# johannah/drqv2

Hardware: AMD Instinct MI355X
Metric: agent updates/sec (batch=256, 9x84x84 obs) (higher is better)
Workload: dtype f32; 1 GPU; cheetah_run batch_size=256/GPU (256 global) 9x84x84 u8 obs, A=6, feature_dim=50, hidden_dim=1024, fp32, use_tb=True; parallelism=dp1, global_batch=256

## Files before the change

drqv2_amd/csrc/conv1aug.hip:

```cpp
#include "common.h"
#include "internal.h"
#include "replay_device.h"
#include "wino_u.h"

namespace {

constexpr int H = 84, C = 9, PAD = 4, S = 92, HW = H * H;
constexpr int HO = 41, PO = HO * HO;
constexpr int NBAND = 5;
constexpr int MAXR = 9;
constexpr int NROWS = 2 * MAXR + 1;
constexpr int SROWS = NROWS + 2;
constexpr int XPL = 42;
constexpr int XPITCH = 2 * XPL;
constexpr int HQ = H / 4;
constexpr int CP = 5, NS = CP * 9;
constexpr int XS_FLOATS = C * NROWS * XPITCH;
constexpr int U8_DWORDS = C * SROWS * HQ;
constexpr int NDMA = (U8_DWORDS + 63) / 64;
constexpr int U8_ALLOC = NDMA * 64;
constexpr int NTHR = 256;
constexpr int NWAVE = NTHR / 64;
constexpr int MAXU = 64;
constexpr int FG = 3, GC = C / FG;
constexpr int LDS_BYTES = (XS_FLOATS + U8_ALLOC + H + (2 + FG) * MAXU) * 4;
static_assert(2 * LDS_BYTES <= 160 * 1024, "two workgroups share a CU's LDS");

struct Conv1AugArgs {
  const uint8_t* obs[2];
  const long* fidx[2];
  const uint8_t* ring_first;
  long ring_R, ring_N;
  const float* shift[2];
  const float* base;
  const float* w;
  const float* bias;
  float* xaug;
  float* y;
  int n, n_store;
  unsigned y_bytes;
  int stagger;
  const float* wino_w[3];
  float* wino_u;
  int n_rider;
};

typedef float f32x2 __attribute__((ext_vector_type(2)));
typedef __bf16 bf16x8_c1 __attribute__((ext_vector_type(8)));
typedef unsigned u32x4_c1 __attribute__((ext_vector_type(4)));
typedef unsigned u32x2_c1 __attribute__((ext_vector_type(2)));

__device__ __forceinline__ unsigned pack_bf16_c1(float lo, float hi) {
  typedef __bf16 bf16x2_c1 __attribute__((ext_vector_type(2)));
  const bf16x2_c1 v = {(__bf16)lo, (__bf16)hi};
  return __builtin_bit_cast(unsigned, v);
}

__device__ __forceinline__ float div255(float v) {
  const float r = 1.0f / 255.0f;
  const float q = __fmul_rn(v, r);
  const float e = __fmaf_rn(-q, 255.0f, v);
  return __fmaf_rn(e, r, q);
}

template <bool BF = false, bool YN = false>
__global__ __launch_bounds__(NTHR, 2 * NTHR / 256) void conv1_aug_kernel(Conv1AugArgs a) {
#pragma clang fp contract(off)
  extern __shared__ __attribute__((aligned(16))) float smem[];
  typedef __attribute__((address_space(3))) void* lds_ptr_t;
  typedef const __attribute__((address_space(1))) void* glb_ptr_t;
  float* xs = smem;
  unsigned* u8w = reinterpret_cast<unsigned*>(smem + XS_FLOATS);
  const uint8_t* u8b = reinterpret_cast<const uint8_t*>(u8w);
  float* bg = smem + XS_FLOATS + U8_ALLOC;
  float* shs = bg + H;
  int* fof = reinterpret_cast<int*>(shs + 2 * MAXU);
  const int tid = threadIdx.x;
  const int lane = tid & 63, wid = __builtin_amdgcn_readfirstlane(tid >> 6);
  const int col = lane & 31, half = lane >> 5;
  if ((int)blockIdx.x < a.n_rider) {
    const int job = blockIdx.x;
    wino_u_image<false>(a.wino_w[job >> 1], job & 1, smem, a.wino_u + (size_t)job * 16384, tid);
    return;
  }
  const int bid = (int)blockIdx.x - a.n_rider;
  const int units = 2 * a.n * NBAND;
  const int G = (int)gridDim.x - a.n_rider;

  if (tid < H) bg[tid] = a.base[tid];
  if (tid >= 128 && tid < 128 + MAXU) {
    const int k = tid - 128, uu = bid + k * G;
    if (uu < units) {
      const int f = uu / NBAND;
      const int view = f >= a.n ? 1 : 0, fb = f - view * a.n;
      shs[2 * k + 0] = a.shift[view][2 * fb + 0];
      shs[2 * k + 1] = a.shift[view][2 * fb + 1];
      const long f0 = a.fidx[view] ? a.fidx[view][fb] : fb;
      if (a.ring_first) {
        const long S = a.ring_R * a.ring_N;
        long sl[FG];
        ring_stack_slots(a.ring_first, a.ring_R, a.ring_N, f0 < 0 ? 0 : (f0 < S ? f0 : S - 1), sl);
#pragma unroll
        for (int g = 0; g < FG; ++g) fof[FG * k + g] = (int)sl[g];
      } else {
#pragma unroll
        for (int g = 0; g < FG; ++g) fof[FG * k + g] = (int)(FG * f0 + g);
      }
    }
  }
  float wreg[NS];
#pragma unroll
  for (int c = 0; c < CP; ++c)
#pragma unroll
    for (int t = 0; t < 9; ++t) {
      const int cin = 2 * c + half;
      wreg[c * 9 + t] = cin < C ? a.w[(col * C + cin) * 9 + t] : 0.f;
    }
  bf16x8_c1 wfb[9];
  if constexpr (BF) {
#pragma unroll
    for (int t = 0; t < 9; ++t) {
      float wv[8];
#pragma unroll
      for (int j = 0; j < 8; ++j) {
        const int cin = 8 * half + j;
        wv[j] = cin < C ? a.w[(col * C + (cin < C ? cin : 0)) * 9 + t] : 0.f;
      }
      const u32x4_c1 pk = {pack_bf16_c1(wv[0], wv[1]), pack_bf16_c1(wv[2], wv[3]), pack_bf16_c1(wv[4], wv[5]),
                           pack_bf16_c1(wv[6], wv[7])};
      wfb[t] = __builtin_bit_cast(bf16x8_c1, pk);
    }
  }
  float breg[16];
#pragma unroll
  for (int r = 0; r < 16; ++r) breg[r] = a.bias[(r & 3) + 8 * (r >> 2) + 4 * half];
  const __amdgpu_buffer_rsrc_t yrsrc = __builtin_amdgcn_make_buffer_rsrc((void*)a.y, 0, a.y_bytes, 0x00020000);
  __syncthreads();

  const float sc = (float)(2.0 / (double)S);
  auto cl = [&](int v) { v -= PAD; return v < 0 ? 0 : (v > H - 1 ? H - 1 : v); };
  auto coordv = [&](int k, float sh, float& fl) {
    const float g = bg[k] + sh;
    const float v = ((g + 1.f) * (float)S - 1.f) / 2.f;
    fl = floorf(v);
    return v;
  };

  struct Unit {
    int f, r0, R, i0, nr, sy_lo, nsrc, fo[FG];
    float shx, shy;
  };
  auto make_unit = [&](int k) {
    const int u = bid + k * G;
    Unit q;
    q.f = u / NBAND;
    const int band = u - q.f * NBAND;
    q.r0 = band == 0 ? 0 : 9 + 8 * (band - 1);
    q.R = band == 0 ? 9 : 8;
    q.i0 = 2 * q.r0;
    q.nr = 2 * q.R + 1 + (band == NBAND - 1 ? 1 : 0);
    q.shx = shs[2 * k + 0] * sc;
    q.shy = shs[2 * k + 1] * sc;
#pragma unroll
    for (int g = 0; g < FG; ++g) q.fo[g] = fof[FG * k + g];
    float fa, fbb;
    coordv(q.i0, q.shy, fa);
    coordv(q.i0 + q.nr - 1, q.shy, fbb);
    q.sy_lo = cl((int)fa);
    q.nsrc = cl((int)fbb + 1) - q.sy_lo + 1;
    return q;
  };
  auto dma_src = [&](const Unit& q) {
    const int view = q.f >= a.n ? 1 : 0;
    const uint8_t* src3[FG];
#pragma unroll
    for (int g = 0; g < FG; ++g) src3[g] = a.obs[view] + (long)q.fo[g] * GC * HW;
    for (int k = wid; k < NDMA; k += NWAVE) {
      int e = k * 64 + lane;
      e = e < U8_DWORDS ? e : U8_DWORDS - 1;
      const int rowid = e / HQ, qd = e - rowid * HQ;
      const int ch = rowid / SROWS, r = rowid - ch * SROWS;
      const int rr = r < q.nsrc ? r : q.nsrc - 1;
      const int grp = ch / GC;
      const uint8_t* src = grp == 0 ? src3[0] : (grp == 1 ? src3[1] : src3[2]);
      const unsigned* g = reinterpret_cast<const unsigned*>(src + (ch - grp * GC) * HW + (q.sy_lo + rr) * H) + qd;
      __builtin_amdgcn_global_load_lds((glb_ptr_t)g, (lds_ptr_t)(u8w + k * 64), 4, 0, 0);
    }
  };

  const int nmine = bid < units ? (units - 1 - bid) / G + 1 : 0;
  Unit cur{};
  if (nmine > 0) {
    cur = make_unit(0);
    dma_src(cur);
  }
  if (a.stagger) {
    const unsigned hwid = __builtin_amdgcn_s_getreg((4 << 0) | (0 << 6) | (31 << 11));
    if (hwid & 1u) {
      for (int q = 0; q < a.stagger; ++q) __builtin_amdgcn_s_sleep(127);
    }
  }
  for (int k = 0; k < nmine; ++k) {
    asm volatile("s_waitcnt vmcnt(0)" ::: "memory");
    __syncthreads();

    {
      const bool store = cur.f < a.n_store;
      const __amdgpu_buffer_rsrc_t xrs = __builtin_amdgcn_make_buffer_rsrc(
          (void*)(a.xaug + (long)cur.f * C * HW), 0, store ? (unsigned)(C * HW * 4) : 0u, 0x00020000);
      constexpr int RPP = NTHR / H;
      const int j = tid % H, r3 = tid / H;
      if (r3 < RPP) {
        float fx;
        const float ix = coordv(j, cur.shx, fx);
        const int x0 = (int)fx;
        const float wx1 = ix - fx, wx0 = (fx + 1.f) - ix;
        const bool okx0 = x0 >= 0 && x0 < S, okx1 = x0 + 1 >= 0 && x0 + 1 < S;
        const int sx0 = cl(x0), sx1 = cl(x0 + 1);
        const int xcol = (j & 1) * XPL + (j >> 1);
        for (int il = r3; il < cur.nr; il += RPP) {
          const int i = cur.i0 + il;
          float fy;
          const float iy = coordv(i, cur.shy, fy);
          const int y0 = (int)fy;
          const float wy1 = iy - fy, wy0 = (fy + 1.f) - iy;
          const bool oky0 = y0 >= 0 && y0 < S, oky1 = y0 + 1 >= 0 && y0 + 1 < S;
          const int sy0 = cl(y0), sy1 = cl(y0 + 1);
          const float w00 = okx0 && oky0 ? wx0 * wy0 : 0.f, w01 = okx1 && oky0 ? wx1 * wy0 : 0.f;
          const float w10 = okx0 && oky1 ? wx0 * wy1 : 0.f, w11 = okx1 && oky1 ? wx1 * wy1 : 0.f;
          const int o00 = (sy0 - cur.sy_lo) * H + sx0, o01 = (sy0 - cur.sy_lo) * H + sx1;
          const int o10 = (sy1 - cur.sy_lo) * H + sx0, o11 = (sy1 - cur.sy_lo) * H + sx1;
          const int xo = il * XPITCH + xcol;
          const int go = (i * H + j) * 4;
          uint8_t tap[C][4];
#pragma unroll
          for (int ch = 0; ch < C; ++ch) {
            const uint8_t* s8 = u8b + ch * SROWS * H;
            tap[ch][0] = s8[o00]; tap[ch][1] = s8[o01]; tap[ch][2] = s8[o10]; tap[ch][3] = s8[o11];
          }
          const f32x2 W00 = {w00, w00}, W01 = {w01, w01}, W10 = {w10, w10}, W11 = {w11, w11};
          const f32x2 R255 = {1.0f / 255.0f, 1.0f / 255.0f}, N255 = {-255.0f, -255.0f}, MH = {-0.5f, -0.5f};
#pragma unroll
          for (int cp = 0; cp < C / 2; ++cp) {
            const int c0 = 2 * cp, c1 = 2 * cp + 1;
            f32x2 p0 = (f32x2){(float)tap[c0][0], (float)tap[c1][0]} * W00;
            f32x2 p1 = (f32x2){(float)tap[c0][1], (float)tap[c1][1]} * W01;
            f32x2 p2 = (f32x2){(float)tap[c0][2], (float)tap[c1][2]} * W10;
            f32x2 p3 = (f32x2){(float)tap[c0][3], (float)tap[c1][3]} * W11;
            asm volatile("" : "+v"(p0), "+v"(p1), "+v"(p2), "+v"(p3));
            f32x2 v = p0 + p1;
            asm volatile("" : "+v"(v));
            v = v + p2;
            asm volatile("" : "+v"(v));
            v = v + p3;
            asm volatile("" : "+v"(v));
            f32x2 q = v * R255;
            asm volatile("" : "+v"(q));
            const f32x2 e = __builtin_elementwise_fma(q, N255, v);
            q = __builtin_elementwise_fma(e, R255, q);
            asm volatile("" : "+v"(q));
            q = q + MH;
            xs[c0 * NROWS * XPITCH + xo] = q[0];
            xs[c1 * NROWS * XPITCH + xo] = q[1];
            __builtin_amdgcn_raw_buffer_store_b32(__float_as_uint(q[0]), xrs, go, c0 * HW * 4, 0);
            __builtin_amdgcn_raw_buffer_store_b32(__float_as_uint(q[1]), xrs, go, c1 * HW * 4, 0);
          }
          {
            constexpr int ch = C - 1;
            float p0 = (float)tap[ch][0] * w00, p1 = (float)tap[ch][1] * w01, p2 = (float)tap[ch][2] * w10,
                  p3 = (float)tap[ch][3] * w11;
            asm volatile("" : "+v"(p0), "+v"(p1), "+v"(p2), "+v"(p3));
            float v = p0 + p1;
            v = v + p2;
            v = v + p3;
            v = __fsub_rn(div255(v), 0.5f);
            xs[ch * NROWS * XPITCH + xo] = v;
            __builtin_amdgcn_raw_buffer_store_b32(__float_as_uint(v), xrs, go, ch * HW * 4, 0);
          }
        }
      }
    }
    __syncthreads();

    const Unit done = cur;
    if (k + 1 < nmine) {
      cur = make_unit(k + 1);
      dma_src(cur);
    }

    const int npix = done.R * HO;
    const int ntiles = (npix + 31) >> 5;
    auto load_group = [&](float (&dst)[9], const float* xb, int c) {
      const int ch = (c == CP - 1) ? (C - 1) : 2 * c + half;
      const float* xc = xb + ch * (NROWS * XPITCH);
#pragma unroll
      for (int ky = 0; ky < 3; ++ky) {
        dst[ky * 3 + 0] = xc[ky * XPITCH];
        dst[ky * 3 + 1] = xc[ky * XPITCH + XPL];
        dst[ky * 3 + 2] = xc[ky * XPITCH + 1];
      }
    };
    for (int tile = wid; tile < (wid >= 4 ? 0 : ntiles); tile += 4) {
      const int p0 = tile * 32 + col;
      const int p = p0 < npix ? p0 : npix - 1;
      const int oyl = p / HO, ox = p - oyl * HO;
      const float* xb = xs + (2 * oyl) * XPITCH + ox;
      f32x16 acc;
#pragma unroll
      for (int r = 0; r < 16; ++r) acc[r] = breg[r];
      if constexpr (BF) {
        const float* xj[8];
#pragma unroll
        for (int j = 0; j < 8; ++j) xj[j] = xb + (half ? C - 1 : j) * (NROWS * XPITCH);
#pragma unroll
        for (int t = 0; t < 9; ++t) {
          const int ky = t / 3, kx = t - 3 * ky;
          const int off = ky * XPITCH + (kx == 1 ? XPL : 0) + (kx == 2 ? 1 : 0);
          float v[8];
#pragma unroll
          for (int j = 0; j < 8; ++j) v[j] = xj[j][off];
          const u32x4_c1 pk = {pack_bf16_c1(v[0], v[1]), pack_bf16_c1(v[2], v[3]), pack_bf16_c1(v[4], v[5]),
                               pack_bf16_c1(v[6], v[7])};
          acc = __builtin_amdgcn_mfma_f32_32x32x16_bf16(wfb[t], __builtin_bit_cast(bf16x8_c1, pk), acc, 0, 0, 0);
        }
      } else {
      float X[2][9];
      load_group(X[0], xb, 0);
#pragma unroll
      for (int c = 0; c < CP; ++c) {
        acc = __builtin_amdgcn_mfma_f32_32x32x2f32(wreg[c * 9], X[c & 1][0], acc, 0, 0, 0);
        __builtin_amdgcn_sched_barrier(0);
        if (c + 1 < CP) load_group(X[(c + 1) & 1], xb, c + 1);
        __builtin_amdgcn_sched_barrier(0);
#pragma unroll
        for (int t = 1; t < 9; ++t)
          acc = __builtin_amdgcn_mfma_f32_32x32x2f32(wreg[c * 9 + t], X[c & 1][t], acc, 0, 0, 0);
        __builtin_amdgcn_sched_barrier(0);
      }
      }
      const int oy = done.r0 + oyl;
      if constexpr (YN) {
        const int yo = p0 < npix ? (((done.f * HO + oy) * HO + ox) * 16 + half * 2) * 4 : (int)0x80000000u;
#pragma unroll
        for (int g4 = 0; g4 < 4; ++g4) {
          float v[4];
#pragma unroll
          for (int e = 0; e < 4; ++e) v[e] = acc[4 * g4 + e] > 0.f ? acc[4 * g4 + e] : 0.f;
          const u32x2_c1 o = {pack_bf16_c1(v[0], v[1]), pack_bf16_c1(v[2], v[3])};
          __builtin_amdgcn_raw_buffer_store_b64(o, yrsrc, yo, g4 * 16, 0);
        }
        continue;
      }
      const int yoff = p0 < npix ? (((done.f * 32 + 4 * half) * HO + oy) * HO + ox) * 4 : (int)0x80000000u;
#pragma unroll
      for (int r = 0; r < 16; ++r) {
        const float v = acc[r] > 0.f ? acc[r] : 0.f;
        __builtin_amdgcn_raw_buffer_store_b32(__float_as_uint(v), yrsrc, yoff, ((r & 3) + 8 * (r >> 2)) * PO * 4, 0);
      }
    }
  }
}

}

int drq_conv1_aug_fwd_any(int bf_mma, const uint8_t* obs, const float* shift, const uint8_t* obs1, const float* shift1,
                          const float* base_grid, const float* w, const float* bias, float* xaug, float* y, int n,
                          int n_store, hipStream_t st, const float* const* wino_w, float* wino_u, const long* fidx0,
                          const long* fidx1, const uint8_t* ring_first, long ring_R, long ring_N) {
  if (!obs || !shift || !obs1 || !shift1 || !base_grid || !w || !bias || !y || n <= 0 || n_store < 0 || n_store > 2 * n)
    return DRQ_EARG;
  if (n_store > 0 && !xaug) return DRQ_EARG;
  if (((uintptr_t)obs & 3) || ((uintptr_t)obs1 & 3)) return DRQ_EARG;
  if (ring_first && (!fidx0 || !fidx1 || obs != obs1 || ring_R <= 0 || ring_N <= 0 || ring_R > INT32_MAX / ring_N))
    return DRQ_EARG;
  const size_t yb = (size_t)2 * n * 32 * PO * (bf_mma == 2 ? 2 : 4);
  if (yb >= (1ull << 31) || (bf_mma == 2 && ((uintptr_t)y & 15))) return DRQ_EARG;
  Conv1AugArgs a{};
  a.obs[0] = obs; a.obs[1] = obs1;
  a.fidx[0] = fidx0; a.fidx[1] = fidx1;
  a.ring_first = ring_first; a.ring_R = ring_R; a.ring_N = ring_N;
  a.shift[0] = shift; a.shift[1] = shift1;
  a.base = base_grid; a.w = w; a.bias = bias; a.xaug = xaug; a.y = y;
  a.n = n; a.n_store = n_store; a.y_bytes = (unsigned)yb; a.stagger = 1;
  if (wino_w && wino_u) {
    for (int l = 0; l < 3; ++l) a.wino_w[l] = wino_w[l];
    a.wino_u = wino_u;
    a.n_rider = 6;
  }
  static bool attr_set_dev[kMaxDevices] = {};
  bool& attr_set = attr_set_dev[drq_device()];
  if (!attr_set) {
    hipError_t e = hipFuncSetAttribute((const void*)conv1_aug_kernel<false>, hipFuncAttributeMaxDynamicSharedMemorySize,
                                       LDS_BYTES);
    if (e == hipSuccess)
      e = hipFuncSetAttribute((const void*)conv1_aug_kernel<true>, hipFuncAttributeMaxDynamicSharedMemorySize, LDS_BYTES);
    if (e == hipSuccess)
      e = hipFuncSetAttribute((const void*)conv1_aug_kernel<true, true>, hipFuncAttributeMaxDynamicSharedMemorySize,
                              LDS_BYTES);
    if (e != hipSuccess) return (int)e;
    attr_set = true;
  }
  const long units = (long)2 * n * NBAND;
  long blocks = units;
  const long cap = 2L * drq_num_cus();
  if (blocks > cap) blocks = cap;
  if (blocks * MAXU < units) blocks = (units + MAXU - 1) / MAXU;
  blocks += a.n_rider;
  if (bf_mma == 2) hipLaunchKernelGGL((conv1_aug_kernel<true, true>), dim3((unsigned)blocks), dim3(NTHR), LDS_BYTES, st, a);
  else if (bf_mma) hipLaunchKernelGGL((conv1_aug_kernel<true>), dim3((unsigned)blocks), dim3(NTHR), LDS_BYTES, st, a);
  else hipLaunchKernelGGL((conv1_aug_kernel<false>), dim3((unsigned)blocks), dim3(NTHR), LDS_BYTES, st, a);
  DRQ_LAUNCH_CHECK();
  return DRQ_OK;
}

DRQ_API int drq_conv1_aug_fwd(const uint8_t* obs, const float* shift, const uint8_t* obs1, const float* shift1,
                              const float* base_grid, const float* w, const float* bias, float* xaug, float* y, int n,
                              int n_store, hipStream_t st) {
  return drq_conv1_aug_fwd_any(0, obs, shift, obs1, shift1, base_grid, w, bias, xaug, y, n, n_store, st, nullptr, nullptr,
                               nullptr, nullptr, nullptr, 0, 0);
}

DRQ_API int drq_conv1_aug_fwd_indexed(const uint8_t* frames, const long* idx, const float* shift, const uint8_t* frames1,
                                      const long* idx1, const float* shift1, const float* base_grid, const float* w,
                                      const float* bias, float* xaug, float* y, int n, int n_store, hipStream_t st) {
  if (!idx || !idx1) return DRQ_EARG;
  return drq_conv1_aug_fwd_any(0, frames, shift, frames1, shift1, base_grid, w, bias, xaug, y, n, n_store, st, nullptr,
                               nullptr, idx, idx1, nullptr, 0, 0);
}

DRQ_API int drq_conv1_aug_fwd_frames(const uint8_t* frames, const uint8_t* first, long R, long N, const long* idx,
                                     const float* shift, const long* idx1, const float* shift1, const float* base_grid,
                                     const float* w, const float* bias, float* xaug, float* y, int n, int n_store,
                                     hipStream_t st) {
  if (!first || !idx || !idx1) return DRQ_EARG;
  return drq_conv1_aug_fwd_any(0, frames, shift, frames, shift1, base_grid, w, bias, xaug, y, n, n_store, st, nullptr,
                               nullptr, idx, idx1, first, R, N);
}

DRQ_API int drq_conv1_aug_fwd_frames_bf16(const uint8_t* frames, const uint8_t* first, long R, long N, const long* idx,
                                          const float* shift, const long* idx1, const float* shift1,
                                          const float* base_grid, const float* w, const float* bias, float* xaug,
                                          float* y, int n, int n_store, hipStream_t st) {
  if (!first || !idx || !idx1) return DRQ_EARG;
  return drq_conv1_aug_fwd_any(1, frames, shift, frames, shift1, base_grid, w, bias, xaug, y, n, n_store, st, nullptr,
                               nullptr, idx, idx1, first, R, N);
}

DRQ_API int drq_conv1_aug_fwd_bf16(const uint8_t* obs, const float* shift, const uint8_t* obs1, const float* shift1,
                                   const float* base_grid, const float* w, const float* bias, float* xaug, float* y,
                                   int n, int n_store, hipStream_t st) {
  return drq_conv1_aug_fwd_any(1, obs, shift, obs1, shift1, base_grid, w, bias, xaug, y, n, n_store, st, nullptr, nullptr,
                               nullptr, nullptr, nullptr, 0, 0);
}

DRQ_API int drq_conv1_aug_fwd_bf16_nhwc(const uint8_t* obs, const float* shift, const uint8_t* obs1, const float* shift1,
                                        const float* base_grid, const float* w, const float* bias, float* xaug,
                                        void* y_nhwc, int n, int n_store, hipStream_t st) {
  return drq_conv1_aug_fwd_any(2, obs, shift, obs1, shift1, base_grid, w, bias, xaug, (float*)y_nhwc, n, n_store, st,
                               nullptr, nullptr, nullptr, nullptr, nullptr, 0, 0);
}
```

drqv2_amd/replay.py:

```python
import collections
import datetime
import pathlib

import numpy as np
import torch

from . import _lib
from . import episodes as _episodes
from ._lib import launch, ptr
from .checkpoint import check_state, host

ExportReport = collections.namedtuple("ExportReport", "files episodes transitions next_row zero_length headless open short")
ExportReport.__doc__ = """What export_episodes() did: files (the paths written, in order), episodes and transitions (how many
of each they hold), next_row (pass it as start_row next time), and how many runs were left out as zero_length, headless,
open and short (drqv2_amd.episodes.plan_export says what each means)."""
FillReport = collections.namedtuple("FillReport", "episodes transitions rows pad_rows")
FillReport.__doc__ = """What add_episodes() did: episodes and transitions placed, rows added to the ring (T grew by that), and
pad_rows, the reset rows that fill the shorter lanes (counted over all environments)."""


class IndexedBatch(tuple):

    def __new__(cls, frames, obs_idx, action, reward, discount, next_idx):
        self = super().__new__(cls, (obs_idx, action, reward, discount, next_idx))
# ... 98 lines not shown
    if isinstance(priority_alpha, bool) or not (0.0 < a <= 1.0):
        raise ValueError(f"priority_alpha {priority_alpha!r}: None or a float in (0, 1]")
    if not (store.priority_beta >= 0.0) or not (0.0 < store.priority_eps < float("inf")):
        raise ValueError("priority_beta must be >= 0 and priority_eps > 0")
    return a


def _priority_tree(store, slots, alpha):
    _on_gpu(store, "prioritized replay keeps its sum tree")
    store.priority_alpha = alpha
    store.tree_leaves = 1 << max(0, slots - 1).bit_length()
    store.tree = torch.zeros(2 * store.tree_leaves, dtype=torch.float64, device=store.device)
    store.tree[0] = 1.0
    store._pbufs = {}


class BatchIterator:

    def __init__(self, draw, store=None):
        self._draw = draw
        self._store = store
        self._ahead = None
        self._drawn = None

    def __iter__(self):
        return self

    def __next__(self):
        b, self._ahead = self._ahead, None
        return b if b is not None else self._draw()

    def prefetch(self):
        if self._ahead is None:
            self._ahead = self._draw()
            if self._store is not None:
                self._drawn = (self._store.last_index, self._store.last_steps)

    def peek(self):
        self.prefetch()
        return self._ahead

    def state_dict(self):
        store = self._store
        if store is None:
            raise _lib.DrqError("BatchIterator.state_dict(): this iterator was built without a store: only the iterators "
                                "of VecDeviceReplay / VecFrameReplay can be saved")
        sd = {"format": 1, "kind": "BatchIterator", "pending": self._ahead is not None}
        if self._ahead is None:
            return sd
        if not store.indexed:
            raise _lib.DrqError("BatchIterator.state_dict(): a pending materialised batch (indexed=False) cannot be saved")
        if store.device.type == "cuda":
            torch.cuda.synchronize(store.device)
        b = self._ahead
        sd.update(index=host(self._drawn[0]), steps=host(self._drawn[1]), action=host(b[1]), reward=host(b[2]),
                  discount=host(b[3]), prioritized=isinstance(b, PrioritizedBatch))
        if sd["prioritized"]:
            sd.update(weights=host(b.weights), stamp=int(b._stamp))
        return sd

    def load_state_dict(self, sd):
        store = self._store
        if store is None:
            raise _lib.DrqError("BatchIterator.load_state_dict(): this iterator was built without a store")
        check_state(self, sd, kind="BatchIterator")
        if not sd.get("pending"):
            self._ahead = self._drawn = None
            return
        index = sd.get("index")
        if not torch.is_tensor(index) or index.dim() != 2 or index.shape[0] != 3:
            raise ValueError("BatchIterator.load_state_dict(): a pending batch needs its index tensor [3, B]")
        B, per = int(index.shape[1]), bool(sd.get("prioritized"))
        want = {"index": ((3, B), torch.int64), "steps": ((B,), torch.int32), "action": ((B, store.A), torch.float32),
                "reward": ((B, 1), torch.float32), "discount": ((B, 1), torch.float32)}
        if per:
            want["weights"] = ((B,), torch.float32)
        check_state(self, sd, tensors=want, kind="BatchIterator")
        if per != (store.tree is not None) or not store.indexed:
            raise ValueError("BatchIterator.load_state_dict(): the saved batch is "
                             f"{'prioritized' if per else 'uniform'} and indexed, the store is not")
        if B and not (0 <= int(index.min()) and int(index.max()) < store.R * store.N):
            raise ValueError(f"BatchIterator.load_state_dict(): slots outside the ring of {store.R * store.N}")
        dev = store.device
        idx, steps, act, rew, disc = (sd[k].to(dev) for k in ("index", "steps", "action", "reward", "discount"))
        batch = store._batch(per, idx, act, rew, disc)
        if per:
            batch._per(store, idx[2], sd["weights"].to(dev))
            batch._stamp = int(sd["stamp"])
        self._ahead, self._drawn = batch, (idx, steps)
        store.last_index, store.last_steps = idx, steps


class DeviceReplay:
    def __init__(self, capacity_steps, obs_shape, action_dim, nstep, discount, device, seed=None, indexed=False,
                 priority_alpha=None, priority_beta=0.4, priority_eps=1e-6, single_frames=False, check_stacks=True):
        self.device = torch.device(device)
        self.obs_shape = tuple(int(s) for s in obs_shape)
        self.single_frames, self.check_stacks = bool(single_frames), bool(check_stacks)
        if self.single_frames and self.obs_shape != (9, 84, 84):
            raise ValueError(f"obs_shape {self.obs_shape}: a single-frame store stacks three (3, 84, 84) frames")
        self.stack_bytes = int(np.prod(self.obs_shape))
        self.frame_bytes = self.stack_bytes // 3 if self.single_frames else self.stack_bytes
        if self.frame_bytes % 16:
            raise ValueError("frame size must be a multiple of 16 bytes")
        self.A = int(action_dim)
        self.nstep = int(nstep)
        self.gamma = float(discount)
        self.capacity = int(capacity_steps)
        dev = self.device
        self.frames = torch.empty((self.capacity, self.frame_bytes), dtype=torch.uint8, device=dev)
        self.action = torch.zeros((self.capacity, self.A), dtype=torch.float32, device=dev)
        self.reward = torch.zeros((self.capacity,), dtype=torch.float32, device=dev)
        self.discount = torch.ones((self.capacity,), dtype=torch.float32, device=dev)
        self.first = torch.zeros((self.capacity,), dtype=torch.uint8, device=dev) if self.single_frames else None
        self.episodes = []
        self._head = 0
        self.rng = np.random.RandomState(seed)
        self._out = {}
        self.indexed = bool(indexed)
        self._ibufs = {}
        self._placements = 0
        self.n_valid = 0
        alpha = _priority_args(self, priority_alpha, priority_beta, priority_eps)
        if alpha is not None:
            _priority_tree(self, self.capacity, alpha)

    def __len__(self):
        return sum(n - 1 for _, n in self.episodes)

    def _place(self, n):
        if n > self.capacity:
            raise ValueError(f"episode of {n} steps exceeds the store ({self.capacity})")
        start = self._head if self._head + n <= self.capacity else 0
        end = start + n
        clear = lambda e: e[0] + e[1] <= start or e[0] >= end
        evicted = [e for e in self.episodes if not clear(e)]
        self.episodes = [e for e in self.episodes if clear(e)]
        self._head = end
        return start, evicted

    def _fill(self, lo, hi, mode):
        launch("drq_per_fill", ptr(self.tree), self.tree_leaves, lo, hi, mode, device=self.device)

    def _place_priorities(self, start, n, evicted):
        for s, m in evicted:
            self._fill(s, s + m, 0)
        self._fill(start, start + n, 0)
        if n - 1 >= self.nstep:
            self._fill(start + 1, start + n - self.nstep + 1, 1)
        self.n_valid = sum(m - self.nstep for _, m in self.episodes if m - 1 >= self.nstep)

    def add_episode(self, episode):
        if self.single_frames:
            obs = newest_frames(episode["observation"], self.check_stacks)
        else:
            obs = np.ascontiguousarray(episode["observation"])
            if obs.dtype != np.uint8 or int(np.prod(obs.shape[1:])) != self.frame_bytes:
                raise ValueError("observation must be uint8 frames of the configured shape")
        n = obs.shape[0]
        start, evicted = self._place(n)
        sl = slice(start, start + n)
        dev = self.device
        self.frames[sl].copy_(torch.from_numpy(obs.reshape(n, self.frame_bytes)), non_blocking=False)
        if self.single_frames:
            flags = np.zeros(n, np.uint8)
            flags[0] = 1
            self.first[sl].copy_(torch.from_numpy(flags))
        self.action[sl].copy_(torch.from_numpy(np.asarray(episode["action"], np.float32).reshape(n, self.A)))
        self.reward[sl].copy_(torch.from_numpy(np.asarray(episode["reward"], np.float32).reshape(n)))
        self.discount[sl].copy_(torch.from_numpy(np.asarray(episode["discount"], np.float32).reshape(n)))
        self.episodes.append([start, n])
        self._placements += 1
        if self.tree is not None:
            self._place_priorities(start, n, evicted)
        return start

    def draw_positions(self, batch_size):
        ok = [(s, n) for s, n in self.episodes if n - 1 >= self.nstep]
        if not ok:
            raise _lib.DrqError("replay: no stored episode is at least nstep long")
        starts = np.array([s for s, _ in ok], np.int64)
        lens = np.array([n - 1 for _, n in ok], np.int64)
        e = self.rng.randint(0, len(ok), size=batch_size)
        idx = (self.rng.random_sample(batch_size) * (lens[e] - self.nstep + 1)).astype(np.int64) + 1
        return starts[e] + idx

    def gather(self, pos):
        _on_gpu(self, "replay batch assembly runs")
        if not torch.is_tensor(pos):
            pos = torch.from_numpy(np.ascontiguousarray(pos, np.int64))
        pos = pos.to(self.device, non_blocking=True)
        B = pos.numel()
        out = self._out.get(B)
        if out is None:
            dev = self.device
            out = (torch.empty((B, self.stack_bytes), dtype=torch.uint8, device=dev),
                   torch.empty((B, self.A), dtype=torch.float32, device=dev),
                   torch.empty((B, 1), dtype=torch.float32, device=dev),
                   torch.empty((B, 1), dtype=torch.float32, device=dev),
                   torch.empty((B, self.stack_bytes), dtype=torch.uint8, device=dev))
            self._out = {B: out}
        obs, act, rew, disc, nxt = out
        shp = (B,) + self.obs_shape
        if self.single_frames:
            launch("drq_nstep_gather_frames", ptr(self.frames), ptr(self.first), self.capacity, ptr(self.action),
                   ptr(self.reward), ptr(self.discount), ptr(pos), B, self.A, self.frame_bytes, self.nstep, self.gamma,
                   ptr(obs), ptr(act), ptr(rew), ptr(disc), ptr(nxt), device=self.device)
            return obs.view(shp), act, rew, disc, nxt.view(shp)
        launch("drq_nstep_gather", ptr(self.frames), ptr(self.action), ptr(self.reward), ptr(self.discount), ptr(pos),
               B, self.A, self.frame_bytes, self.nstep, self.gamma, ptr(obs), ptr(act), ptr(rew), ptr(disc), ptr(nxt),
               device=self.device)
        return obs.view(shp), act, rew, disc, nxt.view(shp)

    def gather_indexed(self, pos):
        _on_gpu(self, "replay batch assembly runs")
        pos = np.ascontiguousarray(pos, np.int64)
        B = pos.size
        dev = self.device
        f = lambda *sh: torch.empty(sh, dtype=torch.float32, device=dev)
        idx, act, rew, disc, host = _rotating(self._ibufs, B, lambda: (
            torch.empty((3, B), dtype=torch.int64, device=dev), f(B, self.A), f(B, 1), f(B, 1),
            torch.empty((3, B), dtype=torch.int64).pin_memory()))
        h = host.numpy()
        h[0], h[1], h[2] = pos - 1, pos + self.nstep - 1, pos
        idx.copy_(host, non_blocking=True)
        launch("drq_nstep_gather", ptr(self.frames), ptr(self.action), ptr(self.reward), ptr(self.discount),
               ptr(idx[2]), B, self.A, self.frame_bytes, self.nstep, self.gamma, None, ptr(act), ptr(rew), ptr(disc),
               None, device=self.device)
        return self._batch(False, idx, act, rew, disc)

    def _batch(self, prioritized, idx, act, rew, disc):
        if self.single_frames:
            return (_PrioritizedFrames if prioritized else FrameBatch)(self.frames, idx[0], act, rew, disc, idx[1],
                                                                       self.first, self.capacity, 1)
        return (_PrioritizedIndexed if prioritized else IndexedBatch)(self.frames, idx[0], act, rew, disc, idx[1])

    def sample_prioritized(self, batch_size):
        if self.n_valid <= 0:
            raise _lib.DrqError("replay: no stored episode is at least nstep long")
        B = int(batch_size)
        dev = self.device
        f = lambda *sh: torch.empty(sh, dtype=torch.float32, device=dev)
        idx, u, w, host, rows = _rotating(self._pbufs, B, lambda: (
            torch.empty((3, B), dtype=torch.int64, device=dev), torch.empty((B,), dtype=torch.float64, device=dev),
            f(B), torch.empty((B,), dtype=torch.float64).pin_memory(),
            (f(B, self.A), f(B, 1), f(B, 1)) if self.indexed else None))
        host.numpy()[:] = self.rng.random_sample(B)
        u.copy_(host, non_blocking=True)
        launch("drq_per_sample", ptr(self.tree), self.tree_leaves, ptr(u), B, self.nstep, self.n_valid,
               float(self.priority_beta), ptr(idx), ptr(w), device=self.device)
        if self.indexed:
            act, rew, disc = rows
            launch("drq_nstep_gather", ptr(self.frames), ptr(self.action), ptr(self.reward), ptr(self.discount),
                   ptr(idx[2]), B, self.A, self.frame_bytes, self.nstep, self.gamma, None, ptr(act), ptr(rew), ptr(disc),
                   None, device=self.device)
            batch = self._batch(True, idx, act, rew, disc)
        else:
            batch = _PrioritizedTuple(self.gather(idx[2]))
        return batch._per(self, idx[2], w)

    def _stamp_now(self):
        return self._placements

    def _update_priorities(self, batch, td_abs):
        if batch._stamp != self._placements:
            return
        pos = batch._pos
        B = _td_rows(pos, td_abs)
        launch("drq_per_update", ptr(self.tree), self.tree_leaves, ptr(pos), ptr(td_abs), B, self.priority_alpha,
               self.priority_eps, device=self.device)

    def sample(self, batch_size):
        if self.tree is not None:
            return self.sample_prioritized(batch_size)
        pos = self.draw_positions(batch_size)
        return self.gather_indexed(pos) if self.indexed else self.gather(pos)

    def __iter__(self):
        return BatchIterator(lambda: self.sample(self.batch_size))

    batch_size = 256


class VecDeviceReplay:

    K = 4
    _draw_copies = True

    def __init__(self, rows, num_envs, obs_shape, action_dim, nstep, discount, device, seed=None, indexed=True,
                 guard_rows=8, priority_alpha=None, priority_beta=0.4, priority_eps=1e-6):
        self.device = torch.device(device)
        self.obs_shape = tuple(int(s) for s in obs_shape)
        self.slot_shape = self.obs_shape
        self.frame_bytes = self.stack_bytes = int(np.prod(self.obs_shape))
        self.R, self.N, self.A = int(rows), int(num_envs), int(action_dim)
        self.nstep, self.gamma, self.guard_rows = int(nstep), float(discount), int(guard_rows)
        if self.frame_bytes <= 0 or self.frame_bytes % 16:
            raise ValueError("frame size must be a multiple of 16 bytes")
        if self.N < 1 or self.A < 1 or self.nstep < 1 or self.guard_rows < 0:
            raise ValueError("num_envs, action_dim and nstep must be >= 1, guard_rows >= 0")
        if self.R < self.nstep + self.guard_rows + 2:
            raise ValueError(f"rows {self.R}: at least nstep + guard_rows + 2 = {self.nstep + self.guard_rows + 2}")
        dev, S = self.device, self.R * self.N
        self.frames = torch.empty((S, self.frame_bytes), dtype=torch.uint8, device=dev)
        self.action = torch.zeros((S, self.A), dtype=torch.float32, device=dev)
        self.reward = torch.zeros((S,), dtype=torch.float32, device=dev)
        self.discount = torch.ones((S,), dtype=torch.float32, device=dev)
        self.first = torch.ones((S,), dtype=torch.uint8, device=dev)
        self.T = 0
        self.rng = np.random.RandomState(seed)
        self.indexed = bool(indexed)
        self.last_steps = None
        self.last_index = None
        self._stage = None
        self._bufs = {}
        self._frames_out = {}
        alpha = _priority_args(self, priority_alpha, priority_beta, priority_eps)
        if alpha is not None:
            if not self.indexed:
                raise ValueError("prioritized sampling on the ring yields indexed batches: indexed=True required")
            _priority_tree(self, S, alpha)

    def bounds(self):
        return max(1, self.T - self.R + 1 + self.guard_rows), self.T - self.nstep

    def _batch(self, prioritized, idx, act, rew, disc):
        return (_PrioritizedIndexed if prioritized else IndexedBatch)(self.frames, idx[0], act, rew, disc, idx[1])

    def __len__(self):
        lo, hi = self.bounds()
        return max(0, hi - lo + 1) * self.N

    def _row(self, x, name, shapes, dtypes):
        t = torch.from_numpy(np.ascontiguousarray(x)) if isinstance(x, np.ndarray) else x
        if not torch.is_tensor(t):
            raise ValueError(f"add(): {name} must be a numpy array or a tensor")
        if tuple(t.shape) not in shapes:
            raise ValueError(f"add(): {name} of shape {shapes[0]} required, got {tuple(t.shape)}")
        if t.dtype not in dtypes:
            raise ValueError(f"add(): {name} must be {dtypes[0]}, got {t.dtype}")
        if t.device.type != "cpu" and t.device != self._device_index():
            raise ValueError(f"add(): {name} is on {t.device}, the store on {self.device}")
        if t.dtype != dtypes[0]:
            t = t.to(dtypes[0])
        return t.contiguous()

    def _device_index(self):
        d = self.device
        if d.type == "cuda" and d.index is None:
            return torch.device("cuda", torch.cuda.current_device())
        return d

    def _staged(self, k, t):
        if self._stage is None:
            N, A, fb, dev = self.N, self.A, self.frame_bytes, self.device
            mk = lambda shape, dt: (torch.empty(shape, dtype=dt).pin_memory(), torch.empty(shape, dtype=dt, device=dev))
            self._stage = [mk((N, fb), torch.uint8), mk((N, A), torch.float32), mk((N,), torch.float32),
                           mk((N,), torch.float32), mk((N,), torch.uint8)]
        pin, dv = self._stage[k]
        pin.copy_(t.reshape(pin.shape))
        dv.copy_(pin, non_blocking=False)
        return dv

    def add(self, obs, action, reward, discount, first=None):
        N = self.N
        args = [self._row(obs, "obs", [(N,) + self.slot_shape, (N, self.frame_bytes)], (torch.uint8,))]
        args += self._scalar_rows(action, reward, discount, first)
        self._write_row(args, self._staged, lambda src: launch(
            "drq_vec_add", ptr(self.frames), ptr(self.action), ptr(self.reward), ptr(self.discount), ptr(self.first),
            self.R, N, self.A, self.frame_bytes, self.T, *(ptr(t) for t in src), device=self.device))

    def _scalar_rows(self, action, reward, discount, first):
        N, f32 = self.N, (torch.float32, torch.float64)
        return [self._row(action, "action", [(N, self.A)], f32),
                self._row(reward, "reward", [(N,), (N, 1)], f32),
                self._row(discount, "discount", [(N,), (N, 1)], f32),
                None if first is None else self._row(first, "first", [(N,)], (torch.uint8, torch.bool))]

    def _write_row(self, args, staged, write):
        N = self.N
        _on_gpu(self, "the step-major replay lives")
        with torch.cuda.device(self.device):
            src = [t if t is None or t.is_cuda else staged(k, t) for k, t in enumerate(args)]
            write(src)
            for t in src:
                if t is not None:
                    t.record_stream(torch.cuda.current_stream())
            self._row_added()

    def _row_added(self):
        self.T += 1
        if self.tree is not None:
            lo, hi = self.bounds()
            enter, leave = (hi if hi >= lo else -1), (lo - 1 if lo >= 2 else -1)
            if enter >= 0 or leave >= 0:
                launch("drq_vec_per_advance", ptr(self.tree), self.tree_leaves, ptr(self.first), self.R, self.N, self.T,
                       enter, leave, device=self.device)

    def sample(self, batch_size):
        _on_gpu(self, "the step-major replay lives")
        lo, hi = self.bounds()
        if hi < lo:
            raise _lib.DrqError(f"replay: {self.T} rows added, no drawable row yet (nstep {self.nstep})")
        if self.tree is not None:
            return self._sample_prioritized(int(batch_size), lo, hi)
        B, K, dev = int(batch_size), self.K, self.device
        f = lambda *sh: torch.empty(sh, dtype=torch.float32, device=dev)
        idx, act, rew, disc, steps, u, host = _rotating(self._bufs, B, lambda: (
            torch.empty((3, B), dtype=torch.int64, device=dev), f(B, self.A), f(B, 1), f(B, 1),
            torch.empty((B,), dtype=torch.int32, device=dev), torch.empty((B, K), dtype=torch.float64, device=dev),
            torch.empty((B, K), dtype=torch.float64).pin_memory()))
        host.numpy()[:] = self.rng.random_sample((B, K))
        u.copy_(host, non_blocking=True)
        obs = nxt = None
        if not self.indexed:
            out = self._frames_out.get(B)
            if out is None:
                out = tuple(torch.empty((B, self.stack_bytes), dtype=torch.uint8, device=dev) for _ in range(2))
                self._frames_out = {B: out}
            obs, nxt = out
        copies = not self.indexed and self._draw_copies
        launch("drq_vec_sample", ptr(self.first), ptr(self.action), ptr(self.reward), ptr(self.discount), self.R, self.N,
               self.A, self.frame_bytes, lo, hi, ptr(u), B, K, self.nstep, self.gamma, ptr(idx), ptr(act), ptr(rew),
               ptr(disc), ptr(steps), ptr(self.frames) if copies else None, ptr(obs) if copies else None,
               ptr(nxt) if copies else None, device=dev)
        self.last_steps, self.last_index = steps, idx
        batch = self._batch(False, idx, act, rew, disc)
        if self.indexed:
            return batch
        if not copies:
            return batch.materialize(self.obs_shape, (obs, nxt))
        shp = (B,) + self.obs_shape
        return obs.view(shp), act, rew, disc, nxt.view(shp)

    def _sample_prioritized(self, B, lo, hi):
        dev = self.device
        f = lambda *sh: torch.empty(sh, dtype=torch.float32, device=dev)
        idx, act, rew, disc, steps, w, u, host = _rotating(self._pbufs, B, lambda: (
            torch.empty((3, B), dtype=torch.int64, device=dev), f(B, self.A), f(B, 1), f(B, 1),
            torch.empty((B,), dtype=torch.int32, device=dev), f(B), torch.empty((B,), dtype=torch.float64, device=dev),
            torch.empty((B,), dtype=torch.float64).pin_memory()))
        host.numpy()[:] = self.rng.random_sample(B)
        u.copy_(host, non_blocking=True)
        launch("drq_vec_per_sample", ptr(self.tree), self.tree_leaves, ptr(self.first), ptr(self.action),
               ptr(self.reward), ptr(self.discount), self.R, self.N, self.A, self.T, lo, hi, ptr(u), B, self.nstep,
               self.gamma, float(self.priority_beta), ptr(idx), ptr(act), ptr(rew), ptr(disc), ptr(steps), ptr(w),
               device=dev)
        self.last_steps, self.last_index = steps, idx
        return self._batch(True, idx, act, rew, disc)._per(self, idx[2], w)

    def _stamp_now(self):
        return self.T

    def _update_priorities(self, batch, td_abs):
        if self.T - batch._stamp >= self.guard_rows:
            return
        pos = batch._pos
        B = _td_rows(pos, td_abs)
        lo, hi = self.bounds()
        launch("drq_vec_per_update", ptr(self.tree), self.tree_leaves, ptr(self.first), self.R, self.N, self.T, lo, hi,
               ptr(pos), ptr(td_abs), B, self.priority_alpha, self.priority_eps, device=self.device)

    def __iter__(self):
        return BatchIterator(lambda: self.sample(self.batch_size), self)

    batch_size = 256

    _RING = ("frames", "action", "reward", "discount", "first")

    def _config(self):
        return {"R": self.R, "N": self.N, "A": self.A, "slot_shape": tuple(self.slot_shape), "nstep": self.nstep,
                "gamma": self.gamma, "guard_rows": self.guard_rows, "indexed": self.indexed,
                "priority_alpha": self.priority_alpha, "priority_eps": self.priority_eps}

    def state_dict(self, frames=True):
        if self.device.type == "cuda":
            torch.cuda.synchronize(self.device)
        live = min(self.T, self.R) * self.N
        name, key, pos, has_gauss, cached = self.rng.get_state()
        sd = {"format": 1, "kind": type(self).__name__, "config": self._config(), "T": self.T,
              "priority_beta": self.priority_beta, "live_slots": live, "ring": bool(frames),
              "rng": (name, torch.from_numpy(key.astype(np.int64)), int(pos), int(has_gauss), float(cached))}
        if frames:
            for n in self._RING:
                sd[n] = host(getattr(self, n)[:live])
        if self.tree is not None:
            sd["tree"] = host(self.tree)
        return sd

    def load_state_dict(self, sd, frames=True):
        check_state(self, sd, self._config())
        T, live = sd.get("T"), sd.get("live_slots")
        if not isinstance(T, int) or T < 0 or live != min(T, self.R) * self.N:
            raise ValueError(f"{type(self).__name__}.load_state_dict(): T {T!r} and live_slots {live!r} do not fit a ring "
                             f"of {self.R} rows x {self.N}")
        if frames and not sd.get("ring"):
            raise ValueError(f"{type(self).__name__}.load_state_dict(): the state was saved with frames=False and holds no "
                             "ring; load_state_dict(sd, frames=False) restores the rest")
        want = {n: ((live,) + tuple(getattr(self, n).shape[1:]), getattr(self, n).dtype) for n in self._RING} if frames else {}
        if self.tree is not None:
            want["tree"] = self.tree
        check_state(self, sd, tensors=want)
        rng = sd.get("rng")
        if (not isinstance(rng, (tuple, list)) or len(rng) != 5 or not torch.is_tensor(rng[1]) or rng[1].numel() != 624
                or not 0 <= int(rng[2]) <= 624):
            raise ValueError(f"{type(self).__name__}.load_state_dict(): no RandomState in the saved state")
        if frames:
            for n in self._RING:
                getattr(self, n)[:live].copy_(sd[n])
            self.action[live:].zero_()
            self.reward[live:].zero_()
            self.discount[live:].fill_(1.0)
            self.first[live:].fill_(1)
        if self.tree is not None:
            self.tree.copy_(sd["tree"])
        self.T, self.priority_beta = T, float(sd["priority_beta"])
        self.rng.set_state((rng[0], rng[1].numpy().astype(np.uint32), int(rng[2]), int(rng[3]), float(rng[4])))
        self.last_steps = self.last_index = None

    _stack = 1

    def export_episodes(self, directory, start_row=None, include_open=False, min_length=1, chunk_bytes=256 << 20):
        import replay_buffer as RB
        _on_gpu(self, "the step-major replay lives")
        torch.cuda.synchronize(self.device)
        plan = _episodes.plan_export(self.first.cpu().numpy(), self.T, self.R, self.N, start_row, include_open, min_length)
        table = _episodes.export_table(plan.episodes)
        M, A, sb, dev = int(table.shape[0]), self.A, self.stack_bytes, self.device
        directory = pathlib.Path(directory)
        directory.mkdir(parents=True, exist_ok=True)
        idx = max((i for _, i, _ in RB._episode_files(directory)), default=-1) + 1
        files = []
        if M:
            rows = int(max(1, min(M, int(chunk_bytes) // (sb + 4 * A + 20))))
            mk = lambda pin: [torch.empty(s, dtype=d, device=None if pin else dev, pin_memory=pin) for s, d in (
                ((rows, sb), torch.uint8), ((rows, A), torch.float32), ((rows,), torch.float32), ((rows,), torch.float32),
                ((rows, 3), torch.int32))]
            dv, pins, done = mk(False), [mk(True), mk(True)], [None, None]
            state = {"cur": 0, "arrays": None, "idx": idx}
            offsets = np.concatenate([[0], np.cumsum([n + 1 for _, _, n in plan.episodes])])

            def drain(k, m0, m):
                done[k].synchronize()
                obs, act, rew, disc = (t.numpy() for t in pins[k][:4])
                pos = m0
                while pos < m0 + m:
                    j = state["cur"]
                    n = plan.episodes[j][2]
                    if state["arrays"] is None:
                        state["arrays"] = {"observation": np.empty((n + 1,) + self.obs_shape, np.uint8),
                                           "action": np.empty((n + 1, A), np.float32),
                                           "reward": np.empty((n + 1, 1), np.float32),
                                           "discount": np.empty((n + 1, 1), np.float32)}
                    a = pos - int(offsets[j])
                    b = min(int(offsets[j + 1]), m0 + m) - int(offsets[j])
                    s = slice(pos - m0, pos - m0 + b - a)
                    ep = state["arrays"]
                    ep["observation"][a:b] = obs[s].reshape((b - a,) + self.obs_shape)
                    ep["action"][a:b] = act[s]
                    ep["reward"][a:b, 0] = rew[s]
                    ep["discount"][a:b, 0] = disc[s]
                    pos += b - a
                    if b == n + 1:
                        ts = datetime.datetime.now().strftime("%Y%m%dT%H%M%S")
                        fn = directory / f"{ts}_{state['idx']}_{n}.npz"
                        RB.save_episode(ep, fn)
                        files.append(fn)
                        state["cur"], state["arrays"], state["idx"] = j + 1, None, state["idx"] + 1

            with torch.cuda.device(dev):
                stream = torch.cuda.current_stream()
                prev = None
                for c, m0 in enumerate(range(0, M, rows)):
                    k, m = c & 1, min(rows, M - m0)
                    pin = pins[k]
                    pin[4].numpy()[:m] = table[m0:m0 + m]
                    dv[4][:m].copy_(pin[4][:m], non_blocking=True)
                    launch("drq_vec_export_rows", ptr(self.frames), ptr(self.action), ptr(self.reward),
                           ptr(self.discount), self.R, self.N, A, self.frame_bytes, self._stack, ptr(dv[4]), m,
                           ptr(dv[0]), ptr(dv[1]), ptr(dv[2]), ptr(dv[3]), device=dev)
                    for q in range(4):
                        pin[q][:m].copy_(dv[q][:m], non_blocking=True)
                    done[k] = torch.cuda.Event()
                    done[k].record(stream)
                    if prev is not None:
                        drain(*prev)
                    prev = (k, m0, m)
                drain(*prev)
        return ExportReport(files, len(plan.episodes), sum(n for _, _, n in plan.episodes), plan.next_row,
                            plan.zero_length, plan.headless, plan.open, plan.short)

    def _episode_frames(self, obs, check):
        obs = np.asarray(obs)
        if obs.dtype != np.uint8 or obs.ndim < 1 or tuple(obs.shape[1:]) != self.slot_shape:
            raise ValueError(f"uint8 [len + 1, {', '.join(map(str, self.slot_shape))}] required, got {obs.dtype} "
                             f"{list(obs.shape)}")
        return np.ascontiguousarray(obs)

    def _checked_episode(self, ep, name, check):
        def bad(field, why):
            return ValueError(f"add_episodes(): {name}: {field}: {why}")
        for field in ("observation", "action", "reward", "discount"):
            if field not in ep:
                raise bad(field, "the episode has no such field")
        try:
            frame = self._episode_frames(ep["observation"], check)
        except ValueError as e:
# ... 309 lines not shown
```

Before: 974.3 updates/s.

## Vectorize conv1 augment: four pixels per thread via dword LDS reads and byte perms

The bilinear shift-augment stage now assigns each thread a quad of four output columns and one channel group, instead of one column across all channels. It reads source bytes as 32-bit LDS words and extracts the four taps with v_perm selectors. Each channel's outputs go to global memory with one 128-bit buffer store in place of four 32-bit stores. This is meant to cut LDS byte loads, per-pixel coordinate math and store instruction count, at the cost of more registers and a different thread-to-work mapping. The replay frame buffer is also zero-initialized, presumably so the wider dword reads never touch uninitialized bytes.

```diff
diff --git a/drqv2_amd/csrc/conv1aug.hip b/drqv2_amd/csrc/conv1aug.hip
--- a/drqv2_amd/csrc/conv1aug.hip
+++ b/drqv2_amd/csrc/conv1aug.hip
@@ -24,6 +24,7 @@
 constexpr int MAXU = 64;
 constexpr int FG = 3, GC = C / FG;
 constexpr int LDS_BYTES = (XS_FLOATS + U8_ALLOC + H + (2 + FG) * MAXU) * 4;
+static_assert(2 * GC == 6, "stage 2's fences name six chains");
 static_assert(2 * LDS_BYTES <= 160 * 1024, "two workgroups share a CU's LDS");
 
 struct Conv1AugArgs {
@@ -63,6 +64,14 @@
   return __fmaf_rn(e, r, q);
 }
 
+__device__ __forceinline__ unsigned quad_window(const int (&sx)[4], int& a) {
+  a = sx[0] >> 2;
+  unsigned sel = 0;
+#pragma unroll
+  for (int m = 0; m < 4; ++m) sel |= (unsigned)((sx[m] - 4 * a) & 7) << (8 * m);
+  return sel;
+}
+
 template <bool BF = false, bool YN = false>
 __global__ __launch_bounds__(NTHR, 2 * NTHR / 256) void conv1_aug_kernel(Conv1AugArgs a) {
 #pragma clang fp contract(off)
@@ -71,7 +80,6 @@
   typedef const __attribute__((address_space(1))) void* glb_ptr_t;
   float* xs = smem;
   unsigned* u8w = reinterpret_cast<unsigned*>(smem + XS_FLOATS);
-  const uint8_t* u8b = reinterpret_cast<const uint8_t*>(u8w);
   float* bg = smem + XS_FLOATS + U8_ALLOC;
   float* shs = bg + H;
   int* fof = reinterpret_cast<int*>(shs + 2 * MAXU);
@@ -208,17 +216,30 @@
       const bool store = cur.f < a.n_store;
       const __amdgpu_buffer_rsrc_t xrs = __builtin_amdgcn_make_buffer_rsrc(
           (void*)(a.xaug + (long)cur.f * C * HW), 0, store ? (unsigned)(C * HW * 4) : 0u, 0x00020000);
-      constexpr int RPP = NTHR / H;
-      const int j = tid % H, r3 = tid / H;
-      if (r3 < RPP) {
-        float fx;
-        const float ix = coordv(j, cur.shx, fx);
-        const int x0 = (int)fx;
-        const float wx1 = ix - fx, wx0 = (fx + 1.f) - ix;
-        const bool okx0 = x0 >= 0 && x0 < S, okx1 = x0 + 1 >= 0 && x0 + 1 < S;
-        const int sx0 = cl(x0), sx1 = cl(x0 + 1);
-        const int xcol = (j & 1) * XPL + (j >> 1);
-        for (int il = r3; il < cur.nr; il += RPP) {
+      constexpr int NQ = H / 4;
+      constexpr int RPP = NTHR / (NQ * FG);
+      const int r4 = tid / (NQ * FG), rem = tid - r4 * (NQ * FG);
+      const int grp = rem / NQ, qd = rem - grp * NQ;
+      if (r4 < RPP) {
+        f32x2 WX0[2], WX1[2];
+        int sx0[4], sx1[4];
+#pragma unroll
+        for (int m = 0; m < 4; ++m) {
+          float fx;
+          const float ix = coordv(4 * qd + m, cur.shx, fx);
+          const int x0 = (int)fx;
+          const float wx1 = ix - fx, wx0 = (fx + 1.f) - ix;
+          const bool okx0 = x0 >= 0 && x0 < S, okx1 = x0 + 1 >= 0 && x0 + 1 < S;
+          sx0[m] = cl(x0); sx1[m] = cl(x0 + 1);
+          WX0[m >> 1][m & 1] = okx0 ? wx0 : 0.f;
+          WX1[m >> 1][m & 1] = okx1 ? wx1 : 0.f;
+        }
+        int a0, a1;
+        const unsigned sel0 = quad_window(sx0, a0), sel1 = quad_window(sx1, a1);
+        const unsigned* s32 = u8w + grp * GC * SROWS * HQ;
+        float* xg = xs + grp * GC * NROWS * XPITCH + 2 * qd;
+        const int gq = grp * GC * HW * 4 + qd * 16;
+        for (int il = r4; il < cur.nr; il += RPP) {
           const int i = cur.i0 + il;
           float fy;
           const float iy = coordv(i, cur.shy, fy);
@@ -226,56 +247,69 @@
           const float wy1 = iy - fy, wy0 = (fy + 1.f) - iy;
           const bool oky0 = y0 >= 0 && y0 < S, oky1 = y0 + 1 >= 0 && y0 + 1 < S;
           const int sy0 = cl(y0), sy1 = cl(y0 + 1);
-          const float w00 = okx0 && oky0 ? wx0 * wy0 : 0.f, w01 = okx1 && oky0 ? wx1 * wy0 : 0.f;
-          const float w10 = okx0 && oky1 ? wx0 * wy1 : 0.f, w11 = okx1 && oky1 ? wx1 * wy1 : 0.f;
-          const int o00 = (sy0 - cur.sy_lo) * H + sx0, o01 = (sy0 - cur.sy_lo) * H + sx1;
-          const int o10 = (sy1 - cur.sy_lo) * H + sx0, o11 = (sy1 - cur.sy_lo) * H + sx1;
-          const int xo = il * XPITCH + xcol;
-          const int go = (i * H + j) * 4;
-          uint8_t tap[C][4];
-#pragma unroll
-          for (int ch = 0; ch < C; ++ch) {
-            const uint8_t* s8 = u8b + ch * SROWS * H;
-            tap[ch][0] = s8[o00]; tap[ch][1] = s8[o01]; tap[ch][2] = s8[o10]; tap[ch][3] = s8[o11];
+          const float wy0z = oky0 ? wy0 : 0.f, wy1z = oky1 ? wy1 : 0.f;
+          const f32x2 WY0 = {wy0z, wy0z}, WY1 = {wy1z, wy1z};
+          f32x2 W00[2], W01[2], W10[2], W11[2];
+#pragma unroll
+          for (int h = 0; h < 2; ++h) {
+            W00[h] = WX0[h] * WY0; W01[h] = WX1[h] * WY0;
+            W10[h] = WX0[h] * WY1; W11[h] = WX1[h] * WY1;
           }
-          const f32x2 W00 = {w00, w00}, W01 = {w01, w01}, W10 = {w10, w10}, W11 = {w11, w11};
+          const int o0 = (sy0 - cur.sy_lo) * HQ, o1 = (sy1 - cur.sy_lo) * HQ;
+          const int xo = il * XPITCH;
+          const int go = i * H * 4 + gq;
+          unsigned T[GC][4];
+#pragma unroll
+          for (int c = 0; c < GC; ++c) {
+            const unsigned* s = s32 + c * SROWS * HQ;
+            T[c][0] = __builtin_amdgcn_perm(s[o0 + a0 + 1], s[o0 + a0], sel0);
+            T[c][1] = __builtin_amdgcn_perm(s[o0 + a1 + 1], s[o0 + a1], sel1);
+            T[c][2] = __builtin_amdgcn_perm(s[o1 + a0 + 1], s[o1 + a0], sel0);
+            T[c][3] = __builtin_amdgcn_perm(s[o1 + a1 + 1], s[o1 + a1], sel1);
+          }
           const f32x2 R255 = {1.0f / 255.0f, 1.0f / 255.0f}, N255 = {-255.0f, -255.0f}, MH = {-0.5f, -0.5f};
-#pragma unroll
-          for (int cp = 0; cp < C / 2; ++cp) {
-            const int c0 = 2 * cp, c1 = 2 * cp + 1;
-            f32x2 p0 = (f32x2){(float)tap[c0][0], (float)tap[c1][0]} * W00;
-            f32x2 p1 = (f32x2){(float)tap[c0][1], (float)tap[c1][1]} * W01;
-            f32x2 p2 = (f32x2){(float)tap[c0][2], (float)tap[c1][2]} * W10;
-            f32x2 p3 = (f32x2){(float)tap[c0][3], (float)tap[c1][3]} * W11;
+          constexpr int NCH = 2 * GC;
+          f32x2 v[NCH], q[NCH];
+#pragma unroll
+          for (int z = 0; z < NCH; ++z) {
+            const int c = z >> 1, h = z & 1;
+            auto tapf = [&](int t) {
+              return (f32x2){(float)((T[c][t] >> (16 * h)) & 0xffu), (float)((T[c][t] >> (16 * h + 8)) & 0xffu)};
+            };
+            f32x2 p0 = tapf(0) * W00[h];
+            f32x2 p1 = tapf(1) * W01[h];
+            f32x2 p2 = tapf(2) * W10[h];
+            f32x2 p3 = tapf(3) * W11[h];
             asm volatile("" : "+v"(p0), "+v"(p1), "+v"(p2), "+v"(p3));
-            f32x2 v = p0 + p1;
-            asm volatile("" : "+v"(v));
-            v = v + p2;
-            asm volatile("" : "+v"(v));
-            v = v + p3;
-            asm volatile("" : "+v"(v));
-            f32x2 q = v * R255;
-            asm volatile("" : "+v"(q));
-            const f32x2 e = __builtin_elementwise_fma(q, N255, v);
-            q = __builtin_elementwise_fma(e, R255, q);
-            asm volatile("" : "+v"(q));
-            q = q + MH;
-            xs[c0 * NROWS * XPITCH + xo] = q[0];
-            xs[c1 * NROWS * XPITCH + xo] = q[1];
-            __builtin_amdgcn_raw_buffer_store_b32(__float_as_uint(q[0]), xrs, go, c0 * HW * 4, 0);
-            __builtin_amdgcn_raw_buffer_store_b32(__float_as_uint(q[1]), xrs, go, c1 * HW * 4, 0);
+            v[z] = p0 + p1;
+            q[z] = p2;
+            p0 = p3;
+            asm volatile("" : "+v"(v[z]), "+v"(q[z]), "+v"(p0));
+            v[z] = v[z] + q[z];
+            q[z] = p0;
           }
-          {
-            constexpr int ch = C - 1;
-            float p0 = (float)tap[ch][0] * w00, p1 = (float)tap[ch][1] * w01, p2 = (float)tap[ch][2] * w10,
-                  p3 = (float)tap[ch][3] * w11;
-            asm volatile("" : "+v"(p0), "+v"(p1), "+v"(p2), "+v"(p3));
-            float v = p0 + p1;
-            v = v + p2;
-            v = v + p3;
-            v = __fsub_rn(div255(v), 0.5f);
-            xs[ch * NROWS * XPITCH + xo] = v;
-            __builtin_amdgcn_raw_buffer_store_b32(__float_as_uint(v), xrs, go, ch * HW * 4, 0);
+          asm volatile("" : "+v"(v[0]), "+v"(v[1]), "+v"(v[2]), "+v"(v[3]), "+v"(v[4]), "+v"(v[5]));
+#pragma unroll
+          for (int z = 0; z < NCH; ++z) v[z] = v[z] + q[z];
+          asm volatile("" : "+v"(v[0]), "+v"(v[1]), "+v"(v[2]), "+v"(v[3]), "+v"(v[4]), "+v"(v[5]));
+#pragma unroll
+          for (int z = 0; z < NCH; ++z) q[z] = v[z] * R255;
+          asm volatile("" : "+v"(q[0]), "+v"(q[1]), "+v"(q[2]), "+v"(q[3]), "+v"(q[4]), "+v"(q[5]));
+#pragma unroll
+          for (int z = 0; z < NCH; ++z) {
+            const f32x2 e = __builtin_elementwise_fma(q[z], N255, v[z]);
+            q[z] = __builtin_elementwise_fma(e, R255, q[z]);
+          }
+          asm volatile("" : "+v"(q[0]), "+v"(q[1]), "+v"(q[2]), "+v"(q[3]), "+v"(q[4]), "+v"(q[5]));
+#pragma unroll
+          for (int c = 0; c < GC; ++c) {
+            const f32x2 o0 = q[2 * c] + MH, o1 = q[2 * c + 1] + MH;
+            float* xc = xg + c * NROWS * XPITCH + xo;
+            xc[0] = o0[0]; xc[XPL] = o0[1];
+            xc[1] = o1[0]; xc[XPL + 1] = o1[1];
+            const u32x4_c1 st = {__float_as_uint(o0[0]), __float_as_uint(o0[1]), __float_as_uint(o1[0]),
+                                 __float_as_uint(o1[1])};
+            __builtin_amdgcn_raw_buffer_store_b128(st, xrs, go, c * HW * 4, 0);
           }
         }
       }
diff --git a/drqv2_amd/replay.py b/drqv2_amd/replay.py
--- a/drqv2_amd/replay.py
+++ b/drqv2_amd/replay.py
@@ -424,7 +424,7 @@
         if self.R < self.nstep + self.guard_rows + 2:
             raise ValueError(f"rows {self.R}: at least nstep + guard_rows + 2 = {self.nstep + self.guard_rows + 2}")
         dev, S = self.device, self.R * self.N
-        self.frames = torch.empty((S, self.frame_bytes), dtype=torch.uint8, device=dev)
+        self.frames = torch.zeros((S, self.frame_bytes), dtype=torch.uint8, device=dev)
         self.action = torch.zeros((S, self.A), dtype=torch.float32, device=dev)
         self.reward = torch.zeros((S,), dtype=torch.float32, device=dev)
         self.discount = torch.ones((S,), dtype=torch.float32, device=dev)
```

Result: no change. 976.7 updates/s (median of 3 runs) (+0.2%).
